# cmusphinx/pocketsphinx

Measured on NVIDIA H100. Metric: frames/sec senone-eval+Viterbi, higher is better.
Workload: dtype f32->i16/i32

## Files before the change

### pocketsphinx_b200/csrc/psb_hmm.cu

```cuda
#include "psb_hmmctx.cuh"

#include <stdlib.h>
#include <string.h>

#include <algorithm>
#include <type_traits>

#include <vector>


struct psb_phoneloop_s {
    psb_hmmctx_t *c;
    int n_phones, window, beam, pbeam, pip;
    double penalty_weight;
    Stream stream;
    DevBuf<int32_t> d_ssid, d_tmatid;
    DevBuf<uint16_t> d_senid;
};

namespace {

__device__ __forceinline__ void load_hmm(const psb_hmm_t *p, HmmReg &h, int n)
{
#pragma unroll
// ... 354 lines not shown
    if (!p) return;
    cudaSetDevice(p->c->device);
    cudaStreamSynchronize(p->stream);
    delete p;
}

int psb_phoneloop_launch(psb_phoneloop_t *p, const int16_t *d_senscr, const int32_t *d_utt_off, int32_t n_utt,
                         int32_t *d_best, int32_t *d_pen, psb_hmm_t *d_final, psb_hmm_t *d_trace, cudaStream_t st)
{
    const int H = p->n_phones, N = p->c->n_emit;
    size_t smem = ((size_t)(2 * N + 4 + p->window) * H + 64) * sizeof(int);
    PSB_REQUIRE(smem <= 227 * 1024, "phone loop with %d HMMs needs %zu bytes of shared memory (max 227 KB)", H, smem);
    PSB_CUDA(cudaFuncSetAttribute(phoneloop_kernel, cudaFuncAttributeMaxDynamicSharedMemorySize, (int)smem));
    int threads = std::min(1024, roundup(H, 32));
    PlParams P;
    P.n_phones = H; P.window = p->window; P.beam = p->beam; P.pbeam = p->pbeam; P.pip = p->pip;
    P.penalty_weight = p->penalty_weight;
    phoneloop_kernel<<<n_utt, threads, smem, st>>>(d_senscr, d_utt_off, dev_ctx(p->c), P, p->d_senid, p->d_tmatid, p->d_ssid,
                                                   d_best, d_pen, d_final, d_trace);
    PSB_LAUNCH_CHECK();
    return PSB_OK;
}

int psb_phoneloop_n_phones(const psb_phoneloop_t *p) { return p->n_phones; }

extern "C" int psb_phoneloop_run_device(psb_phoneloop_t *p, const int16_t *d_senscr, const int32_t *utt_off,
                                        int32_t n_utt, int32_t *d_best, int32_t *d_pen, psb_hmm_t *final_hmms,
                                        void *batch)
{
    PSB_REQUIRE(p && d_senscr && utt_off && n_utt >= 0, "psb_phoneloop_run_device: bad argument");
    if (n_utt == 0) return PSB_OK;
    int rc = ctx_check_utts("psb_phoneloop_run_device", utt_off, n_utt, d_senscr);
    if (rc) return rc;
    PSB_CUDA(cudaSetDevice(p->c->device));
    cudaStream_t st = batch ? psb_batch_stream((psb_batch_t *)batch) : p->stream;
    DevBuf<int32_t> d_off;
    DevBuf<psb_hmm_t> d_final;
    if ((rc = d_off.reserve((size_t)n_utt + 1))) return rc;
    if (final_hmms && (rc = d_final.reserve((size_t)n_utt * p->n_phones))) return rc;
    PSB_CUDA(cudaMemcpyAsync(d_off, utt_off, (size_t)(n_utt + 1) * 4, cudaMemcpyHostToDevice, st));
    rc = psb_phoneloop_launch(p, d_senscr, d_off, n_utt, d_best, d_pen, d_final, nullptr, st);
    if (!rc && final_hmms) {
        cudaError_t e = cudaMemcpyAsync(final_hmms, d_final, (size_t)n_utt * p->n_phones * sizeof(psb_hmm_t),
                                        cudaMemcpyDeviceToHost, st);
        if (e != cudaSuccess) { psb_set_error("%s", cudaGetErrorString(e)); rc = PSB_ERR_CUDA; }
    }
    cudaStreamSynchronize(st);
    return rc;
}

extern "C" int psb_phoneloop_run_host(psb_phoneloop_t *p, const int16_t *senscr, const int32_t *utt_off, int32_t n_utt,
                                      int32_t *best, int32_t *pen, psb_hmm_t *hmm_trace)
{
    PSB_REQUIRE(p && senscr && utt_off && n_utt >= 0, "psb_phoneloop_run_host: bad argument");
    if (n_utt == 0) return PSB_OK;
    int rc = ctx_check_utts("psb_phoneloop_run_host", utt_off, n_utt, senscr);
    if (rc) return rc;
    PSB_CUDA(cudaSetDevice(p->c->device));
    const size_t total = utt_off[n_utt], H = p->n_phones;
    DevBuf<int16_t> d_scr;
    DevBuf<int32_t> d_off, d_best, d_pen;
    DevBuf<psb_hmm_t> d_tr;
    if ((rc = d_scr.reserve(std::max<size_t>(1, total * p->c->n_sen))) || (rc = d_off.reserve((size_t)n_utt + 1)) ||
        (best && (rc = d_best.reserve(std::max<size_t>(1, total)))) || (pen && (rc = d_pen.reserve(std::max<size_t>(1, total * H)))) ||
        (hmm_trace && (rc = d_tr.reserve(std::max<size_t>(1, total * H)))))
        return rc;
    cudaError_t e = cudaMemcpy(d_scr, senscr, total * p->c->n_sen * 2, cudaMemcpyHostToDevice);
    if (e == cudaSuccess) e = cudaMemcpy(d_off, utt_off, (size_t)(n_utt + 1) * 4, cudaMemcpyHostToDevice);
    if (e == cudaSuccess) {
        rc = psb_phoneloop_launch(p, d_scr, d_off, n_utt, d_best, d_pen, nullptr, d_tr, p->stream);
        if (!rc) e = cudaStreamSynchronize(p->stream);
        if (!rc && e == cudaSuccess && best) e = cudaMemcpy(best, d_best, total * 4, cudaMemcpyDeviceToHost);
        if (!rc && e == cudaSuccess && pen) e = cudaMemcpy(pen, d_pen, total * H * 4, cudaMemcpyDeviceToHost);
        if (!rc && e == cudaSuccess && hmm_trace)
            e = cudaMemcpy(hmm_trace, d_tr, total * H * sizeof(psb_hmm_t), cudaMemcpyDeviceToHost);
    }
    if (e != cudaSuccess) { psb_set_error("psb_phoneloop_run_host: %s", cudaGetErrorString(e)); rc = PSB_ERR_CUDA; }
    return rc;
}

constexpr int HS_V = 4;
constexpr int HS_TS = 512;
constexpr int SWEEP_FR = 4;
constexpr int HS_THREADS = 128;

struct psb_hmmset_s {
    psb_hmmctx_t *c;
    int64_t n_max, n, pitch;
    int32_t n_seg_max, n_seg;
    int64_t max_seg_len;
    bool any_mpx;
    Stream own_stream;
    cudaStream_t stream;
    DevBuf<int32_t> d_i32;
    DevBuf<uint16_t> d_u16;
    DevBuf<uint8_t> d_mpx;
    DevBuf<int64_t> d_seg_off;
    DevBuf<int64_t> d_seg_base;
    DevBuf<psb_hmm_t> d_aos;
    DevBuf<int32_t> d_snap_i32;
    Event ev[2];
};

namespace {

struct HmmSetDev {
    int32_t *i32;
    uint16_t *u16;
    uint8_t *mpx;
    const int64_t *seg_off, *seg_base;
    int64_t pitch;
    int n_seg;
};

static HmmSetDev dev_set(const psb_hmmset_t *s)
{
    HmmSetDev d;
    d.i32 = s->d_i32; d.u16 = s->d_u16; d.mpx = s->d_mpx; d.seg_off = s->d_seg_off; d.seg_base = s->d_seg_base;
    d.pitch = s->pitch; d.n_seg = s->n_seg;
    return d;
}

template <bool TO_SOA>
__global__ void __launch_bounds__(256)
hmmset_convert_kernel(psb_hmm_t *aos, HmmSetDev s, int64_t n, int ns)
{
    const int64_t a = (int64_t)blockIdx.x * blockDim.x + threadIdx.x;
    if (a >= n) return;
    int lo = 0, hi = s.n_seg;
    while (hi - lo > 1) {
        const int mid = (lo + hi) >> 1;
        if (s.seg_off[mid] <= a) lo = mid; else hi = mid;
    }
    const int64_t i = s.seg_base[lo] + (a - s.seg_off[lo]);
    psb_hmm_t *p = aos + a;
    const int64_t b32 = (i / HS_TS) * (int64_t)(2 * ns + 4) * HS_TS + (i % HS_TS);
    const int64_t b16 = (i / HS_TS) * (int64_t)(ns + 2) * HS_TS + (i % HS_TS);
    int32_t *score = s.i32 + b32, *hist = score + ns * HS_TS, *tail = score + 2 * ns * HS_TS;
    uint16_t *senid = s.u16 + b16, *ids = senid + ns * HS_TS;
    if (TO_SOA) {
        for (int k = 0; k < ns; ++k) {
            score[k * HS_TS] = p->score[k];
            hist[k * HS_TS] = p->history[k];
            senid[k * HS_TS] = p->senid[k];
        }
        tail[0] = p->out_score; tail[HS_TS] = p->out_history; tail[2 * HS_TS] = p->bestscore; tail[3 * HS_TS] = p->frame;
        ids[0] = p->ssid; ids[HS_TS] = (uint16_t)p->tmatid;
        s.mpx[i] = p->mpx;
    }
    else {
        for (int k = 0; k < PSB_HMM_MAX_NSTATE; ++k) {
            p->score[k] = k < ns ? score[k * HS_TS] : 0;
            p->history[k] = k < ns ? hist[k * HS_TS] : 0;
            p->senid[k] = k < ns ? senid[k * HS_TS] : 0;
        }
        p->out_score = tail[0]; p->out_history = tail[HS_TS]; p->bestscore = tail[2 * HS_TS]; p->frame = tail[3 * HS_TS];
        p->ssid = ids[0]; p->tmatid = (int16_t)ids[HS_TS];
        p->mpx = s.mpx[i]; p->n_emit_state = (uint8_t)ns;
        p->ctx = nullptr;
    }
}

__global__ void fill_i32_kernel(int32_t *p, int64_t n, int32_t v)
{
    const int64_t i = (int64_t)blockIdx.x * blockDim.x + threadIdx.x;
    if (i < n) p[i] = v;
}

__device__ __forceinline__ int comp(const int4 &v, int q) { return q == 0 ? v.x : q == 1 ? v.y : q == 2 ? v.z : v.w; }
__device__ __forceinline__ void setc(int4 &v, int q, int x)
{
    if (q == 0) v.x = x; else if (q == 1) v.y = x; else if (q == 2) v.z = x; else v.w = x;
}

__device__ __forceinline__ void mbar_init(uint64_t *bar, int count)
{
    asm volatile("mbarrier.init.shared::cta.b64 [%0], %1;" ::"r"((unsigned)__cvta_generic_to_shared(bar)), "r"(count));
}
__device__ __forceinline__ void mbar_expect_tx(uint64_t *bar, unsigned bytes)
{
    asm volatile("mbarrier.arrive.expect_tx.shared::cta.b64 _, [%0], %1;" ::"r"((unsigned)__cvta_generic_to_shared(bar)), "r"(bytes)
                 : "memory");
}
__device__ __forceinline__ void mbar_wait(uint64_t *bar, unsigned parity)
{
    asm volatile(
        "{\n"
        ".reg .pred p;\n"
        "WAIT_%=:\n"
        "mbarrier.try_wait.parity.shared::cta.b64 p, [%0], %1;\n"
        "@p bra DONE_%=;\n"
        "bra WAIT_%=;\n"
        "DONE_%=:\n"
        "}\n" ::"r"((unsigned)__cvta_generic_to_shared(bar)),
        "r"(parity)
        : "memory");
}
__device__ __forceinline__ void tma_bulk_g2s(void *dst, const void *src, unsigned bytes, uint64_t *bar)
{
    asm volatile("cp.async.bulk.shared::cluster.global.mbarrier::complete_tx::bytes [%0], [%1], %2, [%3];" ::"r"(
                     (unsigned)__cvta_generic_to_shared(dst)),
                 "l"(src), "r"(bytes), "r"((unsigned)__cvta_generic_to_shared(bar))
                 : "memory");
}

template <int NS>
__global__ void __launch_bounds__(HS_THREADS, NS == 3 ? 6 : 4)
hmmset_eval_kernel(HmmSetDev s, HmmCtxDev c, const int16_t *__restrict__ senscr, const int64_t *__restrict__ row0,
                   const int32_t *__restrict__ n_rows, int t, int32_t *__restrict__ best_out)
{
    extern __shared__ __align__(16) int16_t srow[];
    __shared__ int red[HS_THREADS / 32];
    const int seg = blockIdx.y;
    if (n_rows && t >= n_rows[seg]) return;
    const int64_t n = s.seg_off[seg + 1] - s.seg_off[seg];
    const int64_t j0 = ((int64_t)blockIdx.x * HS_THREADS + threadIdx.x) * HS_V;
    if ((int64_t)blockIdx.x * HS_THREADS * HS_V >= n) return;
// ... 148 lines not shown
    const int seg = blockIdx.y, tid = threadIdx.x;
    const int64_t n = s.seg_off[seg + 1] - s.seg_off[seg];
    const int64_t j_base = (int64_t)blockIdx.x * THREADS * V;
    const bool cta_empty = j_base >= n;
    if (!BEAM && cta_empty) return;
    int T = n_frames;
    if (n_rows) T = min(T, n_rows[seg]);
    if (T <= 0) return;
    const unsigned my_rank = BEAM ? cluster_ctarank() : 0u, n_rank = BEAM ? cluster_nctarank() : 1u;
    if (BEAM) {
        hist[0][tid] = 0u;
        hist[1][tid] = 0u;
        if (tid == 0) {
            mbar_init(&xbar[0], 1);
            mbar_init(&xbar[1], 1);
            asm volatile("fence.mbarrier_init.release.cluster;" ::: "memory");
        }
    }
    uint8_t *tps = sw_smem + NBUF * (size_t)buf_bytes;
    for (int q = tid; q < n_tmat * NS * (NS + 1); q += THREADS) tps[q] = c.tp[q];

    int sc[V][NS], hi[V][NS], sid[V][NS], osc[V], ohi[V], tmo[V];
    HmmTp3 tk[V];
    bool live[V], act[V], touched[V];
    const int64_t rem64 = n - j_base - tid;
    const int rem = rem64 < 0 ? -1 : rem64 > V * THREADS ? V * THREADS : (int)rem64;
    auto state_i32 = [&](int v) {
        const int64_t j = j_base + (int64_t)v * THREADS + tid;
        const int64_t i = s.seg_base[seg] + (j < n ? j : 0);
        return s.i32 + (i / HS_TS) * (int64_t)(2 * NS + 4) * HS_TS + (i % HS_TS);
    };
#pragma unroll
    for (int v = 0; v < V; ++v) {
        const int64_t j = j_base + (int64_t)v * THREADS + tid;
        live[v] = j < n;
        const int64_t i = s.seg_base[seg] + (live[v] ? j : 0);
        const int64_t b16 = (i / HS_TS) * (int64_t)(NS + 2) * HS_TS + (i % HS_TS);
        const int32_t *p32 = state_i32(v);
        const uint16_t *p16 = s.u16 + b16;
#pragma unroll
        for (int k = 0; k < NS; ++k) {
            sc[v][k] = live[v] ? p32[k * HS_TS] : PSB_WORST_SCORE;
            hi[v][k] = live[v] ? p32[(NS + k) * HS_TS] : -1;
            sid[v][k] = live[v] ? 2 * (int)p16[k * HS_TS] : 0;
        }
        osc[v] = live[v] ? p32[2 * NS * HS_TS] : PSB_WORST_SCORE;
        ohi[v] = live[v] ? p32[(2 * NS + 1) * HS_TS] : -1;
        tmo[v] = live[v] ? (int)(int16_t)p16[(NS + 1) * HS_TS] * NS * (NS + 1) : 0;
        act[v] = BEAM ? (live[v] && p32[(2 * NS + 3) * HS_TS] == frame0) : live[v];
        touched[v] = act[v];
    }
    __syncthreads();
    if (NS == 3) {
#pragma unroll
        for (int v = 0; v < V; ++v) tk[v] = live[v] ? hmm_tp3_decode(tps + tmo[v]) : hmm_tp3_padding();
    }
    const int64_t r0 = row0 ? row0[seg] : seg;
    const int64_t rstep = row0 ? 1 : gridDim.y;
    const size_t row_bytes = (size_t)c.n_sen * 2;
    auto row_addr = [&](int t) { return reinterpret_cast<uintptr_t>(senscr + (size_t)(r0 + (int64_t)t * rstep) * c.n_sen); };
    const int64_t lim = rows_total - 1 - r0;
    const int t_tma = lim <= 0 ? 0 : (int)min((int64_t)T, (lim + rstep - 1) / rstep);
    auto tma_ok = [&](int t) { return t < t_tma; };
    const unsigned a_lo0 = (unsigned)row_addr(0), a_step = (unsigned)((size_t)rstep * row_bytes);
    if (BEAM) cluster_sync_all();
    auto issue = [&](int t) {
        const uintptr_t a = row_addr(t), a16 = a & ~(uintptr_t)15;
        const unsigned bytes = (unsigned)(((a - a16) + row_bytes + 15) & ~(size_t)15);
        mbar_expect_tx(&full[t % NBUF], bytes);
        tma_bulk_g2s(sw_smem + (size_t)(t % NBUF) * buf_bytes, reinterpret_cast<const void *>(a16), bytes, &full[t % NBUF]);
    };
    if (tid == 0) {
        for (int q = 0; q < NBUF; ++q) mbar_init(&full[q], 1);
        asm volatile("fence.mbarrier_init.release.cluster;" ::: "memory");
    }
    __syncthreads();
    if (tid == 0 && !cta_empty)
        for (int q = 0; q < NBUF && q < T; ++q)
            if (tma_ok(q)) issue(q);
    int best_final[V];
#pragma unroll
    for (int v = 0; v < V; ++v) best_final[v] = PSB_WORST_SCORE;

    for (int t = 0; t < T; ++t) {
        const int b = t & 1, rb = t % NBUF;
        unsigned char *buf = sw_smem + (size_t)rb * buf_bytes;
        const int16_t *srow;
        if (BEAM && cta_empty)
            srow = reinterpret_cast<const int16_t *>(buf);
        else if (tma_ok(t)) {
            mbar_wait(&full[rb], (unsigned)(t / NBUF) & 1u);
            srow = reinterpret_cast<const int16_t *>(buf + ((a_lo0 + (unsigned)t * a_step) & 15u));
        }
        else {
            const int16_t *g = reinterpret_cast<const int16_t *>(row_addr(t));
            int16_t *d = reinterpret_cast<int16_t *>(buf);
            for (int q = tid; q < c.n_sen; q += THREADS) d[q] = g[q];
            __syncthreads();
            srow = d;
        }
        const unsigned char *srowb = reinterpret_cast<const unsigned char *>(srow);
        auto score_at = [&](int off) { return (int)*reinterpret_cast<const int16_t *>(srowb + off); };
        int best = PSB_WORST_SCORE, cnt = 0;
        bool s1_live = false;
        if (NS == 3 && FAST) {
            bool all = true;
#pragma unroll
            for (int v = 0; v < V; ++v) all &= sc[v][1] - score_at(sid[v][1]) > PSB_WORST_SCORE;
            s1_live = __all_sync(0xffffffffu, all);
        }
        auto frame_steps = [&](auto s1_known) {
#pragma unroll
        for (int v = 0; v < V; ++v) {
            if (BEAM && !act[v]) continue;
            ++cnt;
            int bb;
            if (NS == 3) {
                int (&s3)[3] = *reinterpret_cast<int (*)[3]>(sc[v]);
                int (&h3)[3] = *reinterpret_cast<int (*)[3]>(hi[v]);
                bb = hmm_step_3st_dec<decltype(s1_known)::value>(s3, h3, osc[v], ohi[v], tk[v], score_at(sid[v][0]), score_at(sid[v][1]),
                                      score_at(sid[v][NS > 2 ? 2 : 0]));
            }
            else {
                HmmReg h;
                int obs[PSB_HMM_MAX_NSTATE];
#pragma unroll
                for (int k = 0; k < PSB_HMM_MAX_NSTATE; ++k) {
                    h.score[k] = k < NS ? sc[v][k < NS ? k : 0] : PSB_WORST_SCORE;
                    h.hist[k] = k < NS ? hi[v][k < NS ? k : 0] : -1;
                    h.senid[k] = 0;
                    obs[k] = k < NS ? -score_at(sid[v][k < NS ? k : 0]) : 0;
                }
                h.out_score = osc[v]; h.out_hist = ohi[v]; h.best = PSB_WORST_SCORE;
                bb = hmm_step_5st(h, tps + tmo[v], obs);
#pragma unroll
                for (int k = 0; k < NS; ++k) { sc[v][k] = h.score[k]; hi[v][k] = h.hist[k]; }
                osc[v] = h.out_score; ohi[v] = h.out_hist;
            }
            if (!LIVE_TEST || v * THREADS < rem) best = max(best, bb);
            best_final[v] = bb;
        }
        };
        if (NS == 3 && FAST && s1_live) frame_steps(std::true_type());
        else frame_steps(std::false_type());
        best = __reduce_max_sync(0xffffffffu, best);
        if (BEAM) cnt = __reduce_add_sync(0xffffffffu, cnt);
        const int slot = t % (2 * FR);
        if ((tid & 31) == 0) {
            red[slot][tid >> 5] = best;
            if (BEAM) redc[b][tid >> 5] = cnt;
        }
        if (FR > 1 && t % FR != FR - 1 && t + 1 < T) continue;
        const int tf = t - t % FR;
        __syncthreads();
        if (tid == 0 && !cta_empty)
#pragma unroll 1
            for (int u = tf + NBUF; u <= t + NBUF; ++u)
                if (u < T && tma_ok(u)) issue(u);
        if (tid < 32) {
            if (!BEAM) {
#pragma unroll 1
                for (int u = tf; u <= t; ++u) {
                    int v = tid < THREADS / 32 ? red[u % (2 * FR)][tid] : PSB_WORST_SCORE;
                    v = __reduce_max_sync(0xffffffffu, v);
                    if (tid == 0) atomicMax(best_out + (size_t)u * gridDim.y + seg, v);
                }
            }
            else {
                int v = tid < THREADS / 32 ? red[slot][tid] : PSB_WORST_SCORE;
                v = __reduce_max_sync(0xffffffffu, v);
                int cc = tid < THREADS / 32 ? redc[b][tid] : 0;
                cc = __reduce_add_sync(0xffffffffu, cc);
                if (tid == 0) mbar_expect_tx(&xbar[b], n_rank * 8u);
                if ((unsigned)tid < n_rank)
                    st_async_v2(mapa_shared(&cl_slot[b][my_rank], (unsigned)tid), (unsigned)v, (unsigned)cc,
                                mapa_shared(&xbar[b], (unsigned)tid));
            }
        }
        if (BEAM) {
            mbar_wait(&xbar[b], (unsigned)(t >> 1) & 1u);
            int seg_best = PSB_WORST_SCORE, seg_cnt = 0;
            for (unsigned r = 0; r < n_rank; ++r) {
                const int2 m = cl_slot[b][r];
                seg_best = max(seg_best, m.x);
                seg_cnt += m.y;
            }
            if (my_rank == 0 && tid == 0) {
                best_out[(size_t)t * gridDim.y + seg] = seg_best;
                if (n_active_out) n_active_out[(size_t)t * gridDim.y + seg] = seg_cnt;
            }
            hist[b ^ 1][tid] = 0u;
            int dyn = beam;
            if (maxhmmpf >= 0 && seg_cnt > maxhmmpf) {
                const int bw = -beam / 256;
#pragma unroll
                for (int v = 0; v < V; ++v)
                    if (act[v]) {
                        int bin = (seg_best - best_final[v]) / bw;
                        bin = bin > 255 ? 255 : bin;
                        atomicAdd(&hist[b][bin], 1u);
                    }
                if (tid == 0) found = 256;
                cluster_sync_all();
                unsigned tot = 0;
                for (unsigned r = 0; r < n_rank; ++r) tot += ld_cluster_u32(mapa_shared(&hist[b][tid], r));
                unsigned incl = tot;
#pragma unroll
                for (int o = 1; o < 32; o <<= 1) {
                    const unsigned y = __shfl_up_sync(0xffffffffu, incl, o);
                    if ((tid & 31) >= o) incl += y;
                }
                if ((tid & 31) == 31) scan_w[tid >> 5] = incl;
                __syncthreads();
                for (int w = 0; w < (tid >> 5); ++w) incl += scan_w[w];
                if (incl > (unsigned)maxhmmpf) atomicMin(&found, tid);
                __syncthreads();
                dyn = -(found * bw);
            }
            const int thresh = seg_best + dyn;
#pragma unroll
            for (int v = 0; v < V; ++v)
                if (act[v] && !(best_final[v] > thresh)) {
#pragma unroll
                    for (int k = 0; k < NS; ++k) { sc[v][k] = PSB_WORST_SCORE; hi[v][k] = -1; }
                    osc[v] = PSB_WORST_SCORE; ohi[v] = -1; best_final[v] = PSB_WORST_SCORE;
                    act[v] = false;
                }
        }
    }
    if (BEAM) cluster_sync_all();
#pragma unroll
    for (int v = 0; v < V; ++v) {
        if (!live[v] || !touched[v]) continue;
        int32_t *p32 = state_i32(v);
#pragma unroll
        for (int k = 0; k < NS; ++k) {
            p32[k * HS_TS] = sc[v][k];
            p32[(NS + k) * HS_TS] = hi[v][k];
        }
        p32[2 * NS * HS_TS] = osc[v];
        p32[(2 * NS + 1) * HS_TS] = ohi[v];
        p32[(2 * NS + 2) * HS_TS] = best_final[v];
        if (BEAM) p32[(2 * NS + 3) * HS_TS] = act[v] ? frame0 + T : -1;
    }
}

}

extern "C" void psb_hmmset_free(psb_hmmset_t *s)
{
    if (!s) return;
    cudaSetDevice(s->c->device);
    if (s->stream) cudaStreamSynchronize(s->stream);
    delete s;
}

extern "C" int psb_hmmset_create(psb_hmmctx_t *c, int64_t n_max, int32_t n_seg_max, psb_hmmset_t **out)
{
    PSB_REQUIRE(c && out && n_max > 0 && n_seg_max > 0 && n_seg_max <= 65535, "psb_hmmset_create: bad argument");
    const char *v = getenv("PSB_HMMSET_THREADS");
    PSB_REQUIRE(!v || !strcmp(v, "128"), "psb_hmmset_create: PSB_HMMSET_THREADS=%s; the only accepted value is 128", v);
    PSB_CUDA(cudaSetDevice(c->device));
    std::unique_ptr<psb_hmmset_t> s(new psb_hmmset_t());
    s->c = c; s->n_max = n_max; s->n_seg_max = n_seg_max;
    s->pitch = ((n_max + (int64_t)(HS_V - 1) * n_seg_max + HS_TS - 1) / HS_TS) * HS_TS;
    const int ns = c->n_emit;
    int rc = s->d_i32.reserve((size_t)(2 * ns + 4) * s->pitch);
    if (!rc) rc = s->d_u16.reserve((size_t)(ns + 2) * s->pitch);
    if (!rc) rc = s->d_mpx.reserve((size_t)s->pitch);
    if (!rc) rc = s->d_seg_off.reserve((size_t)n_seg_max + 1);
    if (!rc) rc = s->d_seg_base.reserve((size_t)n_seg_max + 1);
    if (rc) return rc;
    cudaError_t e = s->own_stream.create();
    s->stream = s->own_stream;
    if (e == cudaSuccess) e = s->ev[0].create();
    if (e == cudaSuccess) e = s->ev[1].create();
    if (e != cudaSuccess) {
        psb_set_error("psb_hmmset_create: %s", cudaGetErrorString(e));
        return PSB_ERR_CUDA;
    }
    *out = s.release();
    return PSB_OK;
}

extern "C" int psb_hmmset_use_batch_stream(psb_hmmset_t *s, psb_batch_t *b)
{
    PSB_REQUIRE(s, "psb_hmmset_use_batch_stream: null set");
    PSB_CUDA(cudaStreamSynchronize(s->stream));
    s->stream = b ? psb_batch_stream(b) : s->own_stream;
    return PSB_OK;
}

extern "C" int psb_hmmset_snapshot(psb_hmmset_t *s)
{
    PSB_REQUIRE(s && !s->any_mpx, "psb_hmmset_snapshot: null set or multiplexed instances");
    PSB_CUDA(cudaSetDevice(s->c->device));
    const size_t nb = (size_t)(2 * s->c->n_emit + 4) * s->pitch * 4;
    const int rc = s->d_snap_i32.reserve(nb / 4);
    if (rc) return rc;
    PSB_CUDA(cudaMemcpyAsync(s->d_snap_i32, s->d_i32, nb, cudaMemcpyDeviceToDevice, s->stream));
    return PSB_OK;
}

extern "C" int psb_hmmset_restore(psb_hmmset_t *s)
{
    PSB_REQUIRE(s && s->d_snap_i32, "psb_hmmset_restore: no snapshot");
    PSB_CUDA(cudaSetDevice(s->c->device));
    PSB_CUDA(cudaMemcpyAsync(s->d_i32, s->d_snap_i32, (size_t)(2 * s->c->n_emit + 4) * s->pitch * 4, cudaMemcpyDeviceToDevice, s->stream));
    return PSB_OK;
}

static int hmmset_staging(psb_hmmset_t *s)
{
    return s->d_aos.reserve((size_t)s->n_max);
}

extern "C" int psb_hmmset_upload(psb_hmmset_t *s, const psb_hmm_t *hmms, int64_t n, const int64_t *seg_off, int32_t n_seg)
{
    PSB_REQUIRE(s && n >= 0 && n <= s->n_max && n_seg > 0 && n_seg <= s->n_seg_max && seg_off && (n == 0 || hmms),
                "psb_hmmset_upload: bad argument");
    PSB_REQUIRE(seg_off[0] == 0 && seg_off[n_seg] == n, "psb_hmmset_upload: seg_off must run from 0 to n");
    PSB_CUDA(cudaSetDevice(s->c->device));
    int64_t mx = 0;
    std::vector<int64_t> base((size_t)n_seg + 1);
    base[0] = 0;
    for (int pass = 0; pass < 2; ++pass) {
        const int big = pass == 0 ? HS_TS : HS_V;
        for (int i = 0; i < n_seg; ++i) {
            PSB_REQUIRE(seg_off[i + 1] >= seg_off[i], "psb_hmmset_upload: seg_off not monotone at %d", i);
            const int64_t len = seg_off[i + 1] - seg_off[i];
            const int pad = len >= HS_TS ? big : HS_V;
            mx = std::max<int64_t>(mx, len);
            base[(size_t)i + 1] = base[(size_t)i] + (len + pad - 1) / pad * pad;
        }
        if (base[(size_t)n_seg] <= s->pitch) break;
    }
    PSB_REQUIRE(base[(size_t)n_seg] <= s->pitch, "psb_hmmset_upload: internal capacity exceeded");
    s->any_mpx = false;
    for (int64_t i = 0; i < n; ++i) {
        int rc = validate_hmm(s->c, &hmms[i], (int)i);
        if (rc) return rc;
        s->any_mpx |= hmms[i].mpx != 0;
    }
    int rc = hmmset_staging(s);
    if (rc) return rc;
    s->n = n; s->n_seg = n_seg; s->max_seg_len = mx;
    PSB_CUDA(cudaMemcpyAsync(s->d_seg_off, seg_off, (size_t)(n_seg + 1) * 8, cudaMemcpyHostToDevice, s->stream));
    PSB_CUDA(cudaMemcpyAsync(s->d_seg_base, base.data(), (size_t)(n_seg + 1) * 8, cudaMemcpyHostToDevice, s->stream));
    const int ns = s->c->n_emit;
    const int64_t ni = (int64_t)(2 * ns + 4) * s->pitch;
    fill_i32_kernel<<<(unsigned)((ni + 255) / 256), 256, 0, s->stream>>>(s->d_i32, ni, PSB_WORST_SCORE);
    PSB_LAUNCH_CHECK();
    PSB_CUDA(cudaMemsetAsync(s->d_u16, 0, (size_t)(ns + 2) * s->pitch * 2, s->stream));
    PSB_CUDA(cudaMemsetAsync(s->d_mpx, 0, (size_t)s->pitch, s->stream));
    if (n) {
        PSB_CUDA(cudaMemcpyAsync(s->d_aos, hmms, (size_t)n * sizeof(psb_hmm_t), cudaMemcpyHostToDevice, s->stream));
        hmmset_convert_kernel<true><<<(unsigned)((n + 255) / 256), 256, 0, s->stream>>>(s->d_aos, dev_set(s), n, ns);
        PSB_LAUNCH_CHECK();
    }
    PSB_CUDA(cudaStreamSynchronize(s->stream));
    return PSB_OK;
}

extern "C" int psb_hmmset_download(psb_hmmset_t *s, psb_hmm_t *hmms)
{
    PSB_REQUIRE(s && (s->n == 0 || hmms), "psb_hmmset_download: bad argument");
    if (s->n == 0) return PSB_OK;
    PSB_CUDA(cudaSetDevice(s->c->device));
    int rc = hmmset_staging(s);
    if (rc) return rc;
    hmmset_convert_kernel<false><<<(unsigned)((s->n + 255) / 256), 256, 0, s->stream>>>(s->d_aos, dev_set(s), s->n, s->c->n_emit);
    PSB_LAUNCH_CHECK();
    std::vector<psb_hmm_t> tmp((size_t)s->n);
    PSB_CUDA(cudaMemcpyAsync(tmp.data(), s->d_aos, (size_t)s->n * sizeof(psb_hmm_t), cudaMemcpyDeviceToHost, s->stream));
    PSB_CUDA(cudaStreamSynchronize(s->stream));
    for (int64_t i = 0; i < s->n; ++i) {
        void *ctx = hmms[i].ctx;
        hmms[i] = tmp[(size_t)i];
        hmms[i].ctx = ctx;
    }
    return PSB_OK;
}

extern "C" int psb_hmmset_eval_frames_device(psb_hmmset_t *s, const int16_t *d_senscr, const int64_t *d_row0,
                                             const int32_t *d_n_rows, int32_t n_frames, int32_t *d_best, float *ms)
{
    PSB_REQUIRE(s && d_senscr && d_best && n_frames >= 0, "psb_hmmset_eval_frames_device: bad argument");
    if (ms) *ms = 0.f;
    if (n_frames == 0 || s->n_seg == 0) return PSB_OK;
    PSB_CUDA(cudaSetDevice(s->c->device));
    const int64_t nb = (int64_t)n_frames * s->n_seg;
    fill_i32_kernel<<<(unsigned)((nb + 255) / 256), 256, 0, s->stream>>>(d_best, nb, PSB_WORST_SCORE);
    PSB_LAUNCH_CHECK();
    if (s->n == 0) {
        PSB_CUDA(cudaStreamSynchronize(s->stream));
        return PSB_OK;
    }
    const int tile = HS_THREADS * HS_V;
    const dim3 grid((unsigned)((s->max_seg_len + tile - 1) / tile), (unsigned)s->n_seg);
    const HmmSetDev sd = dev_set(s);
    const HmmCtxDev cd = dev_ctx(s->c);
    const size_t smem = (((size_t)cd.n_sen * 2 + 15) & ~(size_t)15) + 16;
    PSB_REQUIRE(smem <= 200 * 1024, "psb_hmmset: %d senones do not fit the shared-memory score row", cd.n_sen);
    auto launch = [&](auto kern, int t, int32_t *best) {
        kern<<<grid, HS_THREADS, smem, s->stream>>>(sd, cd, d_senscr, d_row0, d_n_rows, t, best);
    };
#define PSB_HS_ATTR(NS) PSB_CUDA(cudaFuncSetAttribute(hmmset_eval_kernel<NS>, cudaFuncAttributeMaxDynamicSharedMemorySize, (int)smem))
    if (smem > 48 * 1024) {
        PSB_HS_ATTR(3); PSB_HS_ATTR(5); PSB_HS_ATTR(0);
    }
#undef PSB_HS_ATTR
    PSB_CUDA(cudaEventRecord(s->ev[0], s->stream));
    for (int t = 0; t < n_frames; ++t) {
        int32_t *best = d_best + (size_t)t * s->n_seg;
        if (cd.n_emit == 3) launch(hmmset_eval_kernel<3>, t, best);
        else if (cd.n_emit == 5) launch(hmmset_eval_kernel<5>, t, best);
        else launch(hmmset_eval_kernel<0>, t, best);
        PSB_LAUNCH_CHECK();
    }
    PSB_CUDA(cudaEventRecord(s->ev[1], s->stream));
    PSB_CUDA(cudaStreamSynchronize(s->stream));
    if (ms) PSB_CUDA(cudaEventElapsedTime(ms, s->ev[0], s->ev[1]));
    return PSB_OK;
}

template <int NS, int V, int THREADS, int FR, bool LIVE_TEST = (NS != 3), bool FAST = (NS == 3)>
static int sweep_launch(psb_hmmset_t *s, const int16_t *d_senscr, int64_t rows_total, const int64_t *d_row0,
                        const int32_t *d_n_rows, int32_t n_frames, int32_t *d_best)
{
    const HmmCtxDev cd = dev_ctx(s->c);
    const int buf_bytes = (int)(((size_t)cd.n_sen * 2 + 32 + 127) & ~(size_t)127);
    const int tp_bytes = s->c->n_tmat * NS * (NS + 1);
    const size_t smem = 2 * FR * (size_t)buf_bytes + tp_bytes;
    PSB_REQUIRE(smem <= 200 * 1024, "psb_hmmset_sweep: %d senones / %d transition matrices do not fit shared memory", cd.n_sen, s->c->n_tmat);
    auto kern = hmmset_sweep_kernel<NS, V, THREADS, false, FR, LIVE_TEST, FAST>;
    PSB_CUDA(cudaFuncSetAttribute(kern, cudaFuncAttributeMaxDynamicSharedMemorySize, (int)smem));
    const dim3 grid((unsigned)((s->max_seg_len + THREADS * V - 1) / (THREADS * V)), (unsigned)s->n_seg);
    PSB_CUDA(cudaEventRecord(s->ev[0], s->stream));
    kern<<<grid, THREADS, smem, s->stream>>>(dev_set(s), cd, d_senscr, (long long)rows_total, d_row0, d_n_rows, n_frames, d_best,
                                            s->c->n_tmat, buf_bytes, 0, 0, -1, nullptr);
    PSB_LAUNCH_CHECK();
    PSB_CUDA(cudaEventRecord(s->ev[1], s->stream));
    return PSB_OK;
}

static int sweep_device(psb_hmmset_t *s, const int16_t *d_senscr, int64_t rows_total, const int64_t *d_row0,
                        const int32_t *d_n_rows, int32_t n_frames, int32_t *d_best, int candidate, float *ms)
{
    PSB_REQUIRE(s && d_senscr && d_best && n_frames >= 0 && rows_total > 0, "psb_hmmset_sweep_device: bad argument");
    const HmmCtxDev cd = dev_ctx(s->c);
    if (s->any_mpx || (cd.n_emit != 3 && cd.n_emit != 5) || (cd.n_sen & 1))
        return psb_hmmset_eval_frames_device(s, d_senscr, d_row0, d_n_rows, n_frames, d_best, ms);
    if (ms) *ms = 0.f;
    if (n_frames == 0 || s->n_seg == 0) return PSB_OK;
    PSB_CUDA(cudaSetDevice(s->c->device));
    const int64_t nb = (int64_t)n_frames * s->n_seg;
    fill_i32_kernel<<<(unsigned)((nb + 255) / 256), 256, 0, s->stream>>>(d_best, nb, PSB_WORST_SCORE);
    PSB_LAUNCH_CHECK();
    if (s->n == 0) {
        if (ms) PSB_CUDA(cudaStreamSynchronize(s->stream));
        return PSB_OK;
    }
    int rc;
    if (cd.n_emit == 5) rc = sweep_launch<5, 4, 512, SWEEP_FR>(s, d_senscr, rows_total, d_row0, d_n_rows, n_frames, d_best);
#ifdef PSB_SWEEP_CANDIDATES
    else if (candidate == 1) rc = sweep_launch<3, 4, 256, 2>(s, d_senscr, rows_total, d_row0, d_n_rows, n_frames, d_best);
    else if (candidate == 2) rc = sweep_launch<3, 4, 512, 1>(s, d_senscr, rows_total, d_row0, d_n_rows, n_frames, d_best);
    else if (candidate == 3) rc = sweep_launch<3, 4, 512, 4, false, false>(s, d_senscr, rows_total, d_row0, d_n_rows, n_frames, d_best);
    else if (candidate == 4) rc = sweep_launch<3, 4, 512, 8>(s, d_senscr, rows_total, d_row0, d_n_rows, n_frames, d_best);
    else if (candidate == 5) rc = sweep_launch<3, 4, 256, 2, true, false>(s, d_senscr, rows_total, d_row0, d_n_rows, n_frames, d_best);
    else if (candidate == 6) rc = sweep_launch<3, 4, 512, 2, true, false>(s, d_senscr, rows_total, d_row0, d_n_rows, n_frames, d_best);
    else if (candidate == 7) rc = sweep_launch<3, 4, 512, 2>(s, d_senscr, rows_total, d_row0, d_n_rows, n_frames, d_best);
    else if (candidate == 8) rc = sweep_launch<3, 4, 256, 4>(s, d_senscr, rows_total, d_row0, d_n_rows, n_frames, d_best);
#endif
    else rc = sweep_launch<3, 4, 512, SWEEP_FR>(s, d_senscr, rows_total, d_row0, d_n_rows, n_frames, d_best);
    (void)candidate;
    if (rc) return rc;
    if (ms) {
        PSB_CUDA(cudaStreamSynchronize(s->stream));
        PSB_CUDA(cudaEventElapsedTime(ms, s->ev[0], s->ev[1]));
    }
    return PSB_OK;
}

extern "C" int psb_hmmset_sweep_device(psb_hmmset_t *s, const int16_t *d_senscr, int64_t rows_total, const int64_t *d_row0,
                                       const int32_t *d_n_rows, int32_t n_frames, int32_t *d_best, float *ms)
{
    return sweep_device(s, d_senscr, rows_total, d_row0, d_n_rows, n_frames, d_best, 0, ms);
}

#ifdef PSB_SWEEP_CANDIDATES
extern "C" int psb_hmmset_sweep_candidate_device(psb_hmmset_t *s, const int16_t *d_senscr, int64_t rows_total, const int64_t *d_row0,
                                                 const int32_t *d_n_rows, int32_t n_frames, int32_t *d_best, int32_t candidate,
                                                 float *ms)
{
    return sweep_device(s, d_senscr, rows_total, d_row0, d_n_rows, n_frames, d_best, candidate, ms);
}
#endif

extern "C" int psb_hmmset_sweep_beam_device(psb_hmmset_t *s, const int16_t *d_senscr, int64_t rows_total, const int64_t *d_row0,
                                            const int32_t *d_n_rows, int32_t n_frames, int32_t frame0, int32_t beam,
                                            int32_t maxhmmpf, int32_t *d_best, int32_t *d_n_active, float *ms)
{
    PSB_REQUIRE(s && d_senscr && d_best && n_frames >= 0 && rows_total > 0, "psb_hmmset_sweep_beam_device: bad argument");
    PSB_REQUIRE(beam < 0 && beam > -0x20000000, "psb_hmmset_sweep_beam_device: the beam is a negative log score (got %d)", beam);
    PSB_REQUIRE(maxhmmpf < 0 || beam <= -256, "psb_hmmset_sweep_beam_device: -maxhmmpf needs a beam of at least 256 score units (bin width -beam/256)");
    const HmmCtxDev cd = dev_ctx(s->c);
    PSB_REQUIRE(!s->any_mpx && (cd.n_emit == 3 || cd.n_emit == 5) && !(cd.n_sen & 1),
                "psb_hmmset_sweep_beam_device: plain 3- or 5-state instances and an even senone count (the fused kernel's shapes)");
    constexpr int THREADS = 256, V = 4;
    const int64_t per_seg = (s->max_seg_len + THREADS * V - 1) / (THREADS * V);
    PSB_REQUIRE(per_seg <= 16, "psb_hmmset_sweep_beam_device: a segment of %lld instances needs %lld CTAs, a cluster holds 16",
                (long long)s->max_seg_len, (long long)per_seg);
    if (ms) *ms = 0.f;
    if (n_frames == 0 || s->n_seg == 0) return PSB_OK;
    PSB_CUDA(cudaSetDevice(s->c->device));
    const int64_t nb = (int64_t)n_frames * s->n_seg;
    fill_i32_kernel<<<(unsigned)((nb + 255) / 256), 256, 0, s->stream>>>(d_best, nb, PSB_WORST_SCORE);
    PSB_LAUNCH_CHECK();
    if (d_n_active) PSB_CUDA(cudaMemsetAsync(d_n_active, 0, (size_t)nb * 4, s->stream));
    if (s->n == 0) {
        if (ms) PSB_CUDA(cudaStreamSynchronize(s->stream));
        return PSB_OK;
    }
    const int buf_bytes = (int)(((size_t)cd.n_sen * 2 + 32 + 127) & ~(size_t)127);
    const int tp_bytes = s->c->n_tmat * cd.n_emit * (cd.n_emit + 1);
    const size_t smem = 6 * (size_t)buf_bytes + tp_bytes;
    PSB_REQUIRE(smem <= 200 * 1024, "psb_hmmset_sweep_beam: %d senones / %d transition matrices do not fit shared memory", cd.n_sen, s->c->n_tmat);
    const HmmSetDev sd = dev_set(s);
    const long long rows_ll = rows_total;
    const int n_tmat = s->c->n_tmat;
    cudaLaunchConfig_t cfg = {};
    cfg.gridDim = dim3((unsigned)std::max<int64_t>(per_seg, 1), (unsigned)s->n_seg);
    cfg.blockDim = dim3(THREADS);
    cfg.dynamicSmemBytes = smem;
    cfg.stream = s->stream;
    cudaLaunchAttribute at[1];
    at[0].id = cudaLaunchAttributeClusterDimension;
    at[0].val.clusterDim.x = cfg.gridDim.x; at[0].val.clusterDim.y = 1; at[0].val.clusterDim.z = 1;
    cfg.attrs = at; cfg.numAttrs = 1;
    PSB_CUDA(cudaEventRecord(s->ev[0], s->stream));
#define PSB_SWEEPB(NS)                                                                                                         \
    do {                                                                                                                       \
        auto kern = hmmset_sweep_kernel<NS, V, THREADS, true>;                                                                 \
        PSB_CUDA(cudaFuncSetAttribute(kern, cudaFuncAttributeMaxDynamicSharedMemorySize, (int)smem));                          \
        if (cfg.gridDim.x > 8) PSB_CUDA(cudaFuncSetAttribute(kern, cudaFuncAttributeNonPortableClusterSizeAllowed, 1));       \
        int n_clusters = 0;                                                                                                    \
        PSB_CUDA(cudaOccupancyMaxActiveClusters(&n_clusters, kern, &cfg));                                                     \
        PSB_REQUIRE(n_clusters > 0, "psb_hmmset_sweep_beam: a cluster of %u CTAs with %zu bytes of shared memory each does not fit the device", \
                    cfg.gridDim.x, smem);                                                                                      \
        PSB_CUDA(cudaLaunchKernelEx(&cfg, kern, sd, cd, d_senscr, rows_ll, d_row0, d_n_rows, (int)n_frames, d_best, n_tmat,   \
                                    buf_bytes, (int)frame0, (int)beam, (int)maxhmmpf, d_n_active));                            \
        PSB_LAUNCH_CHECK();                                                                                                    \
    } while (0)
    if (cd.n_emit == 3) PSB_SWEEPB(3);
    else PSB_SWEEPB(5);
#undef PSB_SWEEPB
    PSB_CUDA(cudaEventRecord(s->ev[1], s->stream));
// ... 849 lines not shown
```

Before: 12.80 million.

## Sort HMMs by first senone per CTA slice and spread per-frame reductions across warps

At load time the host sorts the HMMs within each CTA-sized lane slice of a segment by their first senone id and stores a precomputed slot map. The convert kernels use this map in place of a binary search over segments. The intent is that neighbouring lanes gather nearby senone scores from shared memory, giving fewer bank conflicts and better locality. The sweep kernel also tracks the shared-memory row address as a running 32-bit offset, and in the non-beam path hands each frame's cross-warp max reduction and atomic to its own warp instead of looping in warp 0; the cost is host-side sorting and an extra slot buffer.

```diff
diff --git a/pocketsphinx_b200/csrc/psb_hmm.cu b/pocketsphinx_b200/csrc/psb_hmm.cu
--- a/pocketsphinx_b200/csrc/psb_hmm.cu
+++ b/pocketsphinx_b200/csrc/psb_hmm.cu
@@ -460,6 +460,8 @@
 constexpr int HS_V = 4;
 constexpr int HS_TS = 512;
 constexpr int SWEEP_FR = 4;
+constexpr int SWEEP_THREADS = 512;
+constexpr int HS_LANE_SLICE = SWEEP_THREADS * HS_V;
 constexpr int HS_THREADS = 128;
 
 struct psb_hmmset_s {
@@ -475,6 +477,7 @@
     DevBuf<uint8_t> d_mpx;
     DevBuf<int64_t> d_seg_off;
     DevBuf<int64_t> d_seg_base;
+    DevBuf<int64_t> d_slot;
     DevBuf<psb_hmm_t> d_aos;
     DevBuf<int32_t> d_snap_i32;
     Event ev[2];
@@ -488,29 +491,23 @@
     uint8_t *mpx;
     const int64_t *seg_off, *seg_base;
     int64_t pitch;
-    int n_seg;
 };
 
 static HmmSetDev dev_set(const psb_hmmset_t *s)
 {
     HmmSetDev d;
     d.i32 = s->d_i32; d.u16 = s->d_u16; d.mpx = s->d_mpx; d.seg_off = s->d_seg_off; d.seg_base = s->d_seg_base;
-    d.pitch = s->pitch; d.n_seg = s->n_seg;
+    d.pitch = s->pitch;
     return d;
 }
 
 template <bool TO_SOA>
 __global__ void __launch_bounds__(256)
-hmmset_convert_kernel(psb_hmm_t *aos, HmmSetDev s, int64_t n, int ns)
+hmmset_convert_kernel(psb_hmm_t *aos, HmmSetDev s, const int64_t *__restrict__ slot, int64_t n, int ns)
 {
     const int64_t a = (int64_t)blockIdx.x * blockDim.x + threadIdx.x;
     if (a >= n) return;
-    int lo = 0, hi = s.n_seg;
-    while (hi - lo > 1) {
-        const int mid = (lo + hi) >> 1;
-        if (s.seg_off[mid] <= a) lo = mid; else hi = mid;
-    }
-    const int64_t i = s.seg_base[lo] + (a - s.seg_off[lo]);
+    const int64_t i = slot[a];
     psb_hmm_t *p = aos + a;
     const int64_t b32 = (i / HS_TS) * (int64_t)(2 * ns + 4) * HS_TS + (i % HS_TS);
     const int64_t b16 = (i / HS_TS) * (int64_t)(ns + 2) * HS_TS + (i % HS_TS);
@@ -825,25 +822,24 @@
 #pragma unroll
     for (int v = 0; v < V; ++v) best_final[v] = PSB_WORST_SCORE;
 
-    for (int t = 0; t < T; ++t) {
+    const unsigned smem0 = (unsigned)__cvta_generic_to_shared(sw_smem);
+    const unsigned wid = __reduce_min_sync(0xffffffffu, (unsigned)tid) >> 5;
+    const bool warp0 = wid == 0u;
+    unsigned ubuf = 0u, ua = a_lo0;
+    for (int t = 0; t < T; ++t, ua += a_step, ubuf = ubuf == (NBUF - 1) * (unsigned)buf_bytes ? 0u : ubuf + buf_bytes) {
         const int b = t & 1, rb = t % NBUF;
-        unsigned char *buf = sw_smem + (size_t)rb * buf_bytes;
-        const int16_t *srow;
-        if (BEAM && cta_empty)
-            srow = reinterpret_cast<const int16_t *>(buf);
-        else if (tma_ok(t)) {
+        const unsigned mis = ua & 15u, srow = smem0 + ubuf + mis;
+        if (BEAM && cta_empty) {
+        }
+        else if (tma_ok(t))
             mbar_wait(&full[rb], (unsigned)(t / NBUF) & 1u);
-            srow = reinterpret_cast<const int16_t *>(buf + ((a_lo0 + (unsigned)t * a_step) & 15u));
-        }
         else {
             const int16_t *g = reinterpret_cast<const int16_t *>(row_addr(t));
-            int16_t *d = reinterpret_cast<int16_t *>(buf);
+            int16_t *d = reinterpret_cast<int16_t *>(sw_smem + (size_t)rb * buf_bytes + mis);
             for (int q = tid; q < c.n_sen; q += THREADS) d[q] = g[q];
             __syncthreads();
-            srow = d;
-        }
-        const unsigned char *srowb = reinterpret_cast<const unsigned char *>(srow);
-        auto score_at = [&](int off) { return (int)*reinterpret_cast<const int16_t *>(srowb + off); };
+        }
+        auto score_at = [&](int off) { return (int)*static_cast<const int16_t *>(__cvta_shared_to_generic(srow + (unsigned)off)); };
         int best = PSB_WORST_SCORE, cnt = 0;
         bool s1_live = false;
         if (NS == 3 && FAST) {
@@ -900,25 +896,24 @@
 #pragma unroll 1
             for (int u = tf + NBUF; u <= t + NBUF; ++u)
                 if (u < T && tma_ok(u)) issue(u);
-        if (tid < 32) {
-            if (!BEAM) {
-#pragma unroll 1
-                for (int u = tf; u <= t; ++u) {
-                    int v = tid < THREADS / 32 ? red[u % (2 * FR)][tid] : PSB_WORST_SCORE;
-                    v = __reduce_max_sync(0xffffffffu, v);
-                    if (tid == 0) atomicMax(best_out + (size_t)u * gridDim.y + seg, v);
-                }
-            }
-            else {
-                int v = tid < THREADS / 32 ? red[slot][tid] : PSB_WORST_SCORE;
+        if (!BEAM) {
+            static_assert(FR <= THREADS / 32, "one publishing warp per frame closed by a barrier");
+            if (wid <= (unsigned)(t - tf)) {
+                const int u = tf + (int)wid, lane = tid & 31;
+                int v = lane < THREADS / 32 ? red[u % (2 * FR)][lane] : PSB_WORST_SCORE;
                 v = __reduce_max_sync(0xffffffffu, v);
-                int cc = tid < THREADS / 32 ? redc[b][tid] : 0;
-                cc = __reduce_add_sync(0xffffffffu, cc);
-                if (tid == 0) mbar_expect_tx(&xbar[b], n_rank * 8u);
-                if ((unsigned)tid < n_rank)
-                    st_async_v2(mapa_shared(&cl_slot[b][my_rank], (unsigned)tid), (unsigned)v, (unsigned)cc,
-                                mapa_shared(&xbar[b], (unsigned)tid));
-            }
+                if (lane == 0) atomicMax(best_out + (size_t)u * gridDim.y + seg, v);
+            }
+        }
+        else if (warp0) {
+            int v = tid < THREADS / 32 ? red[slot][tid] : PSB_WORST_SCORE;
+            v = __reduce_max_sync(0xffffffffu, v);
+            int cc = tid < THREADS / 32 ? redc[b][tid] : 0;
+            cc = __reduce_add_sync(0xffffffffu, cc);
+            if (tid == 0) mbar_expect_tx(&xbar[b], n_rank * 8u);
+            if ((unsigned)tid < n_rank)
+                st_async_v2(mapa_shared(&cl_slot[b][my_rank], (unsigned)tid), (unsigned)v, (unsigned)cc,
+                            mapa_shared(&xbar[b], (unsigned)tid));
         }
         if (BEAM) {
             mbar_wait(&xbar[b], (unsigned)(t >> 1) & 1u);
@@ -1013,6 +1008,7 @@
     if (!rc) rc = s->d_mpx.reserve((size_t)s->pitch);
     if (!rc) rc = s->d_seg_off.reserve((size_t)n_seg_max + 1);
     if (!rc) rc = s->d_seg_base.reserve((size_t)n_seg_max + 1);
+    if (!rc) rc = s->d_slot.reserve((size_t)n_max);
     if (rc) return rc;
     cudaError_t e = s->own_stream.create();
     s->stream = s->own_stream;
@@ -1087,9 +1083,20 @@
     }
     int rc = hmmset_staging(s);
     if (rc) return rc;
+    std::vector<int64_t> slot((size_t)n);
+    std::vector<uint32_t> key(HS_LANE_SLICE);
+    for (int g = 0; g < n_seg; ++g)
+        for (int64_t a0 = seg_off[g]; a0 < seg_off[g + 1]; a0 += HS_LANE_SLICE) {
+            const int m = (int)std::min<int64_t>(HS_LANE_SLICE, seg_off[g + 1] - a0);
+            for (int j = 0; j < m; ++j) key[(size_t)j] = (uint32_t)hmms[a0 + j].senid[0] << 16 | (uint32_t)j;
+            std::sort(key.begin(), key.begin() + m);
+            const int64_t i0 = base[(size_t)g] + (a0 - seg_off[g]);
+            for (int r = 0; r < m; ++r) slot[(size_t)(a0 + (key[(size_t)r] & 0xffffu))] = i0 + r;
+        }
     s->n = n; s->n_seg = n_seg; s->max_seg_len = mx;
     PSB_CUDA(cudaMemcpyAsync(s->d_seg_off, seg_off, (size_t)(n_seg + 1) * 8, cudaMemcpyHostToDevice, s->stream));
     PSB_CUDA(cudaMemcpyAsync(s->d_seg_base, base.data(), (size_t)(n_seg + 1) * 8, cudaMemcpyHostToDevice, s->stream));
+    if (n) PSB_CUDA(cudaMemcpyAsync(s->d_slot, slot.data(), (size_t)n * 8, cudaMemcpyHostToDevice, s->stream));
     const int ns = s->c->n_emit;
     const int64_t ni = (int64_t)(2 * ns + 4) * s->pitch;
     fill_i32_kernel<<<(unsigned)((ni + 255) / 256), 256, 0, s->stream>>>(s->d_i32, ni, PSB_WORST_SCORE);
@@ -1098,7 +1105,7 @@
     PSB_CUDA(cudaMemsetAsync(s->d_mpx, 0, (size_t)s->pitch, s->stream));
     if (n) {
         PSB_CUDA(cudaMemcpyAsync(s->d_aos, hmms, (size_t)n * sizeof(psb_hmm_t), cudaMemcpyHostToDevice, s->stream));
-        hmmset_convert_kernel<true><<<(unsigned)((n + 255) / 256), 256, 0, s->stream>>>(s->d_aos, dev_set(s), n, ns);
+        hmmset_convert_kernel<true><<<(unsigned)((n + 255) / 256), 256, 0, s->stream>>>(s->d_aos, dev_set(s), s->d_slot, n, ns);
         PSB_LAUNCH_CHECK();
     }
     PSB_CUDA(cudaStreamSynchronize(s->stream));
@@ -1112,7 +1119,7 @@
     PSB_CUDA(cudaSetDevice(s->c->device));
     int rc = hmmset_staging(s);
     if (rc) return rc;
-    hmmset_convert_kernel<false><<<(unsigned)((s->n + 255) / 256), 256, 0, s->stream>>>(s->d_aos, dev_set(s), s->n, s->c->n_emit);
+    hmmset_convert_kernel<false><<<(unsigned)((s->n + 255) / 256), 256, 0, s->stream>>>(s->d_aos, dev_set(s), s->d_slot, s->n, s->c->n_emit);
     PSB_LAUNCH_CHECK();
     std::vector<psb_hmm_t> tmp((size_t)s->n);
     PSB_CUDA(cudaMemcpyAsync(tmp.data(), s->d_aos, (size_t)s->n * sizeof(psb_hmm_t), cudaMemcpyDeviceToHost, s->stream));
@@ -1205,7 +1212,7 @@
         return PSB_OK;
     }
     int rc;
-    if (cd.n_emit == 5) rc = sweep_launch<5, 4, 512, SWEEP_FR>(s, d_senscr, rows_total, d_row0, d_n_rows, n_frames, d_best);
+    if (cd.n_emit == 5) rc = sweep_launch<5, HS_V, SWEEP_THREADS, SWEEP_FR>(s, d_senscr, rows_total, d_row0, d_n_rows, n_frames, d_best);
 #ifdef PSB_SWEEP_CANDIDATES
     else if (candidate == 1) rc = sweep_launch<3, 4, 256, 2>(s, d_senscr, rows_total, d_row0, d_n_rows, n_frames, d_best);
     else if (candidate == 2) rc = sweep_launch<3, 4, 512, 1>(s, d_senscr, rows_total, d_row0, d_n_rows, n_frames, d_best);
@@ -1216,7 +1223,7 @@
     else if (candidate == 7) rc = sweep_launch<3, 4, 512, 2>(s, d_senscr, rows_total, d_row0, d_n_rows, n_frames, d_best);
     else if (candidate == 8) rc = sweep_launch<3, 4, 256, 4>(s, d_senscr, rows_total, d_row0, d_n_rows, n_frames, d_best);
 #endif
-    else rc = sweep_launch<3, 4, 512, SWEEP_FR>(s, d_senscr, rows_total, d_row0, d_n_rows, n_frames, d_best);
+    else rc = sweep_launch<3, HS_V, SWEEP_THREADS, SWEEP_FR>(s, d_senscr, rows_total, d_row0, d_n_rows, n_frames, d_best);
     (void)candidate;
     if (rc) return rc;
     if (ms) {
```

New measurement: 13.14 million (median of 6 runs). 1.03x the previous value.
